# mrsaraei/ViT-2SPN

Measured on NVIDIA B200. Metric: dual-view SSP pairs/sec, ViT-Tiny b128/GPU, higher is better.
Workload: dtype bf16

## Files before the change

### vit-2spn_b200/csrc/common.cuh

```cuda
#pragma once
#include <cuda_bf16.h>
#include <cuda_fp16.h>
#include <cuda_runtime.h>
#include <stdint.h>
#include <string.h>

#include <utility>

#include "../../include/vit2spn.h"

namespace v2s {

typedef __nv_bfloat16 bf16;
typedef __half f16;
constexpr int AT_F32 = 0, AT_BF16 = 1, AT_F16 = 2;

constexpr int D = V2S_HIDDEN;
constexpr int NT = V2S_TOKENS;
constexpr int NP = V2S_PATCHES;
constexpr int NH = V2S_HEADS;
constexpr int DH = V2S_HEAD_DIM;
constexpr int DF = V2S_MLP;
constexpr int NL = V2S_LAYERS;
constexpr int KPE = V2S_PATCH_K;
// ... 64 lines not shown
      v2s::set_error("%s failed: %s (%s:%d)", #expr, cudaGetErrorString(_e), __FILE__, __LINE__); \
      return 1;                                                                               \
    }                                                                                         \
  } while (0)

#define V2S_LAUNCH_CHECK()                                                                    \
  do {                                                                                        \
    ++v2s::g_launch_count;                                                                    \
    cudaError_t _e = cudaGetLastError();                                                      \
    if (_e != cudaSuccess) {                                                                  \
      v2s::set_error("kernel launch failed: %s (%s:%d)", cudaGetErrorString(_e), __FILE__, __LINE__); \
      return 1;                                                                               \
    }                                                                                         \
  } while (0)

#define V2S_TRY(expr)             \
  do {                            \
    int _r = (expr);              \
    if (_r != 0) return _r;       \
  } while (0)

template <typename... KArgs, typename... Args>
inline cudaError_t launch_pdl(void (*kernel)(KArgs...), dim3 grid, dim3 block, size_t smem, cudaStream_t stream,
                              Args&&... args) {
  cudaLaunchConfig_t cfg;
  memset(&cfg, 0, sizeof(cfg));
  cfg.gridDim = grid; cfg.blockDim = block; cfg.dynamicSmemBytes = smem; cfg.stream = stream;
  cudaLaunchAttribute attr[1];
  attr[0].id = cudaLaunchAttributeProgrammaticStreamSerialization;
  attr[0].val.programmaticStreamSerializationAllowed = 1;
  cfg.attrs = attr; cfg.numAttrs = 1;
  return cudaLaunchKernelEx(&cfg, kernel, std::forward<Args>(args)...);
}

template <typename T> __device__ __forceinline__ float to_f(T v);
template <> __device__ __forceinline__ float to_f<float>(float v) { return v; }
template <> __device__ __forceinline__ float to_f<bf16>(bf16 v) { return __bfloat162float(v); }
template <> __device__ __forceinline__ float to_f<f16>(f16 v) { return __half2float(v); }
template <typename T> __device__ __forceinline__ T from_f(float v);
template <> __device__ __forceinline__ float from_f<float>(float v) { return v; }
template <> __device__ __forceinline__ bf16 from_f<bf16>(float v) { return __float2bfloat16_rn(v); }
template <> __device__ __forceinline__ f16 from_f<f16>(float v) { return __float2half_rn(v); }

__device__ __forceinline__ float warp_sum(float v) {
#pragma unroll
  for (int o = 16; o > 0; o >>= 1) v += __shfl_xor_sync(0xffffffffu, v, o);
  return v;
}
__device__ __forceinline__ float warp_max(float v) {
#pragma unroll
  for (int o = 16; o > 0; o >>= 1) v = fmaxf(v, __shfl_xor_sync(0xffffffffu, v, o));
  return v;
}

__device__ __forceinline__ float gelu_f(float x) { return 0.5f * x * (1.0f + erff(x * 0.70710678118654752f)); }
__device__ __forceinline__ float gelu_grad_f(float x) {
  const float cdf = 0.5f * (1.0f + erff(x * 0.70710678118654752f));
  const float pdf = 0.39894228040143268f * __expf(-0.5f * x * x);
  return cdf + x * pdf;
}

template <typename T> struct GPtr {
  T* p[MAXG];
};

}
// ... 1 lines not shown
```

### vit-2spn_b200/csrc/mlp_tc.cu

```cuda
#include <string.h>

#include "gemm_tc.cuh"
#include "mlp_tc.cuh"
#include "ptx.cuh"
#include "tc_math.cuh"

namespace v2s {

namespace {

constexpr int BM = 128;
constexpr int CW = 64;
constexpr int NCH = DF / CW;
constexpr int KB1 = D / 64;
constexpr int KBLK = BM * 128;
constexpr int A1_BYTES = KB1 * KBLK;
constexpr int SW = 2 * CW;
constexpr int NSC = DF / SW;
constexpr int W_SLOT = 24576;
constexpr int W_SLOTS = 3;
constexpr int OFF_W = A1_BYTES;
constexpr int N_EB = 6;
constexpr int OFF_EB = OFF_W + W_SLOTS * W_SLOT;
constexpr int OFF_BAR = OFF_EB + N_EB * KBLK;
constexpr int SMEM_BYTES = OFF_BAR + 1024 + 1024;
constexpr int TM_ACC2 = 128;
constexpr int N_THREADS = 768;
constexpr int GELU_THREADS = 512;
constexpr int DRAIN_THREADS = 128;
constexpr int XCH = D / 32;
static_assert(SMEM_BYTES <= 232448, "shared-memory budget");
static_assert(OFF_W % 1024 == 0 && OFF_EB % 1024 == 0 && W_SLOT % 1024 == 0, "swizzled tiles need 1024-byte alignment");
static_assert(NCH % 2 == 0, "per-buffer phase bookkeeping assumes an even number of chunks per tile");

struct alignas(64) MlpParams {
  CUtensorMap tmA[MAXG], tmB1[MAXG], tmB2[MAXG];
  CUtensorMap tmH[MAXG];
  CUtensorMap tmU[MAXG];
  CUtensorMap tmRes[MAXG];
  CUtensorMap tmOut[MAXG];
  CUtensorMap tmXn[MAXG];
  const float* b1[MAXG]; const float* b2[MAXG];
  const float* ln_gamma[MAXG]; const float* ln_beta[MAXG]; float* ln_mean[MAXG]; float* ln_rstd[MAXG];
  int has_h[MAXG], has_u[MAXG], has_ln[MAXG];
  int M, tiles_m, total_tiles, late_wait;
  int* err_flag;
  long long* dbg;
};

template <int MODE, typename LP, bool DBG>
__global__ void __launch_bounds__(N_THREADS, 1) mlp_tc_kernel(const __grid_constant__ MlpParams p) {
  extern __shared__ uint8_t smem_raw[];
  uint8_t* smem = reinterpret_cast<uint8_t*>((reinterpret_cast<uintptr_t>(smem_raw) + 1023) & ~uintptr_t(1023));
  uint64_t* a1_full = reinterpret_cast<uint64_t*>(smem + OFF_BAR);
  uint64_t* a1_empty = a1_full + 1;
  uint64_t* w_full = a1_empty + 1;
  uint64_t* w_empty = w_full + W_SLOTS;
  uint64_t* acc1_full = w_empty + W_SLOTS;
  uint64_t* acc1_empty = acc1_full + 2;
  uint64_t* a2_full = acc1_empty + 2;
  uint64_t* a2_free = a2_full + 2;
  uint64_t* u_full = a2_free + 2;
  uint64_t* u_free = u_full + 2;
  uint64_t* acc2_full = u_free + 2;
  uint64_t* acc2_empty = acc2_full + 2;
  uint64_t* rs_full = acc2_empty + 2;
  uint64_t* dst_full = rs_full + 2;
  uint64_t* dbuf_free = dst_full + 2;
  uint32_t* tmem_ptr = reinterpret_cast<uint32_t*>(dbuf_free + 2);

  const int warp = __shfl_sync(0xffffffffu, threadIdx.x >> 5, 0), lane = threadIdx.x & 31;

  if (warp == 0 && lane == 0) {
    for (int g = 0; g * p.tiles_m < p.total_tiles; ++g) {
      ptx::prefetch_tmap(&p.tmA[g]); ptx::prefetch_tmap(&p.tmB1[g]); ptx::prefetch_tmap(&p.tmB2[g]);
    }
  }
  if (warp == 1 && lane == 0) {
    ptx::mbar_init(a1_full, 1); ptx::mbar_init(a1_empty, 1);
    for (int s = 0; s < W_SLOTS; ++s) { ptx::mbar_init(&w_full[s], 1); ptx::mbar_init(&w_empty[s], 1); }
    for (int s = 0; s < 2; ++s) {
      ptx::mbar_init(&acc1_full[s], 1); ptx::mbar_init(&acc1_empty[s], 16);
      ptx::mbar_init(&a2_full[s], GELU_THREADS); ptx::mbar_init(&a2_free[s], 2);
      ptx::mbar_init(&u_full[s], MODE == MLP_FWD ? GELU_THREADS : 1);
      ptx::mbar_init(&u_free[s], MODE == MLP_FWD ? 1 : GELU_THREADS);
      ptx::mbar_init(&acc2_full[s], 1); ptx::mbar_init(&acc2_empty[s], 4);
      ptx::mbar_init(&rs_full[s], 1); ptx::mbar_init(&dst_full[s], DRAIN_THREADS); ptx::mbar_init(&dbuf_free[s], 1);
    }
    ptx::fence_barrier_init();
  }
  if (warp == 2) {
    ptx::tmem_alloc(tmem_ptr, 512);
    ptx::tmem_relinquish();
  }
  ptx::tc_fence_before();
  __syncthreads();
  ptx::tc_fence_after();
  const uint32_t tmem_base = __shfl_sync(0xffffffffu, *tmem_ptr, 0);
  if (!p.late_wait) {
    ptx::pdl_wait();
    ptx::pdl_launch_dependents();
  }

  const int n_my = ((int)blockIdx.x < p.total_tiles) ? (p.total_tiles - 1 - (int)blockIdx.x) / (int)gridDim.x + 1 : 0;
  auto tile_at = [&](int i, int& g, int& mt) {
    const int t = blockIdx.x + i * gridDim.x;
    g = t / p.tiles_m;
    mt = t - g * p.tiles_m;
  };
  uint8_t* const eb = smem + OFF_EB;
  long long tk[8] = {0, 0, 0, 0, 0, 0, 0, 0};
  const long long t_begin = DBG ? clock64() : 0;
#define V2S_WAIT(slot, bar, par, code)                                   \
  do {                                                                  \
    const long long _t0 = DBG ? clock64() : 0;                          \
    ptx::mbar_wait(bar, par, p.err_flag, code);                         \
    if (DBG) tk[slot] += clock64() - _t0;                               \
  } while (0)

  if (warp == 0) {
    int ws = 0; uint32_t wph = 0;
    auto advance = [&]() { if (++ws == W_SLOTS) { ws = 0; wph ^= 1; } };
    auto load_b1 = [&](int g, int k) {
#pragma unroll 1
      for (int kb = 0; kb < KB1; ++kb) {
        ptx::mbar_wait(&w_empty[ws], wph ^ 1, p.err_flag, 41);
        if (ptx::elect_one()) {
          uint8_t* slot = smem + OFF_W + ws * W_SLOT;
          ptx::mbar_arrive_expect_tx(&w_full[ws], SW * 128);
          if (MODE == MLP_FWD) {
            ptx::tma_load_2d(slot, &p.tmB1[g], &w_full[ws], kb * 64, k * SW);
          } else {
            ptx::tma_load_2d(slot, &p.tmB1[g], &w_full[ws], k * SW, kb * 64);
            ptx::tma_load_2d(slot + 8192, &p.tmB1[g], &w_full[ws], k * SW + 64, kb * 64);
          }
        }
        __syncwarp();
        advance();
      }
    };
    auto load_b2 = [&](int g, int j) {
      ptx::mbar_wait(&w_empty[ws], wph ^ 1, p.err_flag, 42);
      if (ptx::elect_one()) {
        uint8_t* slot = smem + OFF_W + ws * W_SLOT;
        ptx::mbar_arrive_expect_tx(&w_full[ws], W_SLOT);
        if (MODE == MLP_FWD) {
          ptx::tma_load_2d(slot, &p.tmB2[g], &w_full[ws], j * CW, 0);
        } else {
          ptx::tma_load_2d(slot, &p.tmB2[g], &w_full[ws], 0, j * CW);
          ptx::tma_load_2d(slot + 8192, &p.tmB2[g], &w_full[ws], 64, j * CW);
          ptx::tma_load_2d(slot + 16384, &p.tmB2[g], &w_full[ws], 128, j * CW);
        }
      }
      __syncwarp();
      advance();
    };
    auto load_a1 = [&](int i) {
      int g, mt;
      tile_at(i, g, mt);
      ptx::mbar_wait(a1_empty, (i & 1) ^ 1, p.err_flag, 43);
      if (ptx::elect_one()) {
        ptx::mbar_arrive_expect_tx(a1_full, A1_BYTES);
#pragma unroll
        for (int kb = 0; kb < KB1; ++kb) ptx::tma_load_2d(smem + kb * KBLK, &p.tmA[g], a1_full, kb * 64, mt * BM);
      }
      __syncwarp();
    };
    const int n_sc = n_my * NSC;
    auto grp = [&](int K) { int g, mt; tile_at(K / NSC, g, mt); return g; };
    if (n_sc > 0) { load_a1(0); load_b1(grp(0), 0); }
#pragma unroll 1
    for (int K = 0; K < n_sc; ++K) {
      if (K >= 1) load_b2(grp(K - 1), 2 * ((K - 1) % NSC) + 1);
      if (K + 1 < n_sc) {
        if ((K + 1) % NSC == 0) load_a1((K + 1) / NSC);
        load_b1(grp(K + 1), (K + 1) % NSC);
      }
      load_b2(grp(K), 2 * (K % NSC));
    }
    if (n_sc > 0) load_b2(grp(n_sc - 1), 2 * ((n_sc - 1) % NSC) + 1);
  } else if (warp == 1) {
    constexpr uint32_t b_mn = (MODE == MLP_BWD) ? 1u : 0u;
    const uint32_t idesc2 = make_idesc_lp(LP::kIdescFmt, BM, D, 0, b_mn);
    const uint32_t sbase = ptx::smem_u32(smem);
    const uint32_t b_lbo = b_mn ? 8192u : 16u, b_step = b_mn ? (2048u >> 4) : (32u >> 4);
    int ws = 0; uint32_t wph = 0;
    auto advance = [&]() { if (++ws == W_SLOTS) { ws = 0; wph ^= 1; } };
    const uint32_t idesc1 = make_idesc_lp(LP::kIdescFmt, BM, SW, 0, b_mn);
    auto stage1 = [&](int K) {
      const int i = K / NSC, k = K - i * NSC;
      V2S_WAIT(0, acc1_empty, (K & 1) ^ 1, 44);
      if (k == 0) V2S_WAIT(1, a1_full, i & 1, 45);
#pragma unroll 1
      for (int kb = 0; kb < KB1; ++kb) {
        V2S_WAIT(2, &w_full[ws], wph, 46);
        ptx::tc_fence_after();
        const uint32_t a_lo = ptx::desc_lo(sbase + kb * KBLK, 16);
        const uint32_t b_lo = ptx::desc_lo(sbase + OFF_W + ws * W_SLOT, b_lbo);
        if (ptx::elect_one()) {
#pragma unroll
          for (int kk = 0; kk < 4; ++kk)
            ptx::umma_bf16_lohi(tmem_base, a_lo + kk * 2, b_lo + kk * b_step, ptx::DESC_HI_SW128_SBO1024, idesc1,
                                (kb > 0 || kk > 0) ? 1u : 0u);
          ptx::umma_commit(&w_empty[ws]);
          if (kb == KB1 - 1) {
            ptx::umma_commit(acc1_full);
            if (k == NSC - 1) ptx::umma_commit(a1_empty);
          }
        }
        __syncwarp();
        advance();
      }
    };
    auto stage2 = [&](int c) {
      const int i = c / NCH, j = c - i * NCH;
      const int s = i & 1, b = c & 1;
      if (j == 0) V2S_WAIT(3, &acc2_empty[s], ((i >> 1) & 1) ^ 1, 47);
      V2S_WAIT(4, &a2_full[b], (c >> 1) & 1, 48);
      V2S_WAIT(5, &w_full[ws], wph, 49);
      ptx::tc_fence_after();
      const uint32_t d_tmem = tmem_base + TM_ACC2 + s * D;
      const uint32_t a_lo = ptx::desc_lo(sbase + OFF_EB + b * KBLK, 16);
      const uint32_t b_lo = ptx::desc_lo(sbase + OFF_W + ws * W_SLOT, b_lbo);
      if (ptx::elect_one()) {
#pragma unroll
        for (int kk = 0; kk < 4; ++kk)
          ptx::umma_bf16_lohi(d_tmem, a_lo + kk * 2, b_lo + kk * b_step, ptx::DESC_HI_SW128_SBO1024, idesc2,
                              (j > 0 || kk > 0) ? 1u : 0u);
        ptx::umma_commit(&w_empty[ws]);
        ptx::umma_commit(&a2_free[b]);
        if (j == NCH - 1) ptx::umma_commit(&acc2_full[s]);
      }
      __syncwarp();
      advance();
    };
    const int n_sc = n_my * NSC;
    if (n_sc > 0) stage1(0);
#pragma unroll 1
    for (int K = 0; K < n_sc; ++K) {
      if (K >= 1) stage2(2 * K - 1);
      if (K + 1 < n_sc) stage1(K + 1);
      stage2(2 * K);
    }
    if (n_sc > 0) stage2(2 * n_sc - 1);
    if (DBG && blockIdx.x == 0 && lane == 0) {
      for (int k = 0; k < 6; ++k) p.dbg[k] = tk[k];
      p.dbg[6] = clock64() - t_begin; p.dbg[7] = n_my;
    }
  } else if (warp == 2) {
    int c = 0, nut = 0;
    const int n_chunks = n_my * NCH;
    auto load_u = [&](int cc) {
      const int ti = cc / NCH, jj = cc - ti * NCH;
      int g2, mt2;
      tile_at(ti, g2, mt2);
      ptx::mbar_arrive_expect_tx(&u_full[cc & 1], KBLK);
      ptx::tma_load_2d(eb + (2 + (cc & 1)) * KBLK, &p.tmU[g2], &u_full[cc & 1], jj * CW, mt2 * BM);
    };
    if (MODE == MLP_BWD && lane == 0) {
      if (n_chunks > 0) load_u(0);
      if (n_chunks > 1) load_u(1);
    }
    __syncwarp();
    for (int i = 0; i < n_my; ++i) {
      int g, mt;
      tile_at(i, g, mt);
      const int m0 = mt * BM;
      const bool has_h = p.has_h[g] != 0, has_u = MODE == MLP_FWD && p.has_u[g] != 0;
      const bool stores = has_h || has_u;
#pragma unroll 1
      for (int j = 0; j < NCH; ++j, ++c) {
        const int b = c & 1;
        if (MODE == MLP_BWD && c + 2 < n_chunks) {
          ptx::mbar_wait(&u_free[b], (c >> 1) & 1, p.err_flag, 53);
          if (lane == 0) load_u(c + 2);
          __syncwarp();
        }
        ptx::mbar_wait(&a2_full[b], (c >> 1) & 1, p.err_flag, 54);
        if (has_u) ptx::mbar_wait(&u_full[b], (nut * (NCH / 2) + (j >> 1)) & 1, p.err_flag, 55);
        if (lane == 0) {
          if (stores) {
            if (has_h) ptx::tma_store_2d(&p.tmH[g], eb + b * KBLK, j * CW, m0);
            if (has_u) ptx::tma_store_2d(&p.tmU[g], eb + (2 + b) * KBLK, j * CW, m0);
            ptx::tma_commit_group();
            if (j > 0) {
              ptx::tma_wait_group_read<1>();
              ptx::mbar_arrive(&a2_free[b ^ 1]);
              if (has_u) ptx::mbar_arrive(&u_free[b ^ 1]);
            }
            if (j == NCH - 1) {
              ptx::tma_wait_group_read<0>();
              ptx::mbar_arrive(&a2_free[b]);
              if (has_u) ptx::mbar_arrive(&u_free[b]);
            }
          } else {
            ptx::mbar_arrive(&a2_free[b]);
          }
        }
        __syncwarp();
      }
      if (has_u) ++nut;
    }
    if (lane == 0) ptx::tma_wait_group<0>();
    __syncwarp();
  } else if (warp == 3) {
    int use0 = 0, use1 = 0;
    auto load_res = [&](int ti, int k) {
      int g2, mt2;
      tile_at(ti, g2, mt2);
      ptx::mbar_arrive_expect_tx(&rs_full[k & 1], KBLK);
      ptx::tma_load_2d(eb + (4 + (k & 1)) * KBLK, &p.tmRes[g2], &rs_full[k & 1], k * 32, mt2 * BM);
    };
    if (MODE == MLP_FWD && n_my > 0 && lane == 0) { load_res(0, 0); load_res(0, 1); }
    __syncwarp();
    for (int i = 0; i < n_my; ++i) {
      int g, mt;
      tile_at(i, g, mt);
      const int m0 = mt * BM;
      const int n_out = MODE == MLP_FWD ? XCH : 0;
      const int n_lp = MODE == MLP_FWD ? (p.has_ln[g] != 0 ? 3 : 0) : 3;
      const int n_all = n_out + n_lp;
#pragma unroll 1
      for (int k = 0; k < n_all; ++k) {
        const int t = k - n_out;
        const int b = (k < n_out ? k : t) & 1;
        ptx::mbar_wait(&dst_full[b], (b ? use1 : use0) & 1, p.err_flag, 57);
        if (lane == 0) {
          if (k < n_out) ptx::tma_store_2d(&p.tmOut[g], eb + (4 + b) * KBLK, k * 32, m0);
          else ptx::tma_store_2d(MODE == MLP_FWD ? &p.tmXn[g] : &p.tmOut[g], eb + (4 + b) * KBLK, t * 64, m0);
          ptx::tma_commit_group();
          ptx::tma_wait_group_read<0>();
          ptx::mbar_arrive(&dbuf_free[b]);
          if (MODE == MLP_FWD) {
            if (k + 2 < n_out) load_res(i, k + 2);
            else if (i + 1 < n_my) {
              const bool last_use = n_lp == 0 ? true : (b == 0 ? t == 2 : t == 1);
              if (last_use) load_res(i + 1, b);
            }
          }
        }
        __syncwarp();
        use0 += b ^ 1; use1 += b;
      }
    }
    if (lane == 0) ptx::tma_wait_group<0>();
    __syncwarp();
  } else if (warp >= 4 && warp < 20) {
    const int q = warp & 3;
    const int cq = (warp - 4) >> 2;
    const int row = q * 32 + lane;
    const int rx = row & 7;
    const uint32_t tl = tmem_base + ((uint32_t)(q * 32) << 16);
    const uint32_t eb_row = ptx::smem_u32(eb) + row * 128;
    const uint32_t pc0 = ((2 * cq) ^ rx) << 4, pc1 = ((2 * cq + 1) ^ rx) << 4;
    int c = 0, nut = 0;
    uint32_t rr[32];
    for (int i = 0; i < n_my; ++i) {
      int g, mt;
      tile_at(i, g, mt);
      const bool has_u = MODE == MLP_FWD && p.has_u[g] != 0;
#pragma unroll 1
      for (int j = 0; j < NCH; ++j, ++c) {
        const int b = c & 1;
        uint4 ux0, ux1;
        if (MODE == MLP_BWD) {
          V2S_WAIT(0, &u_full[b], (c >> 1) & 1, 61);
          ux0 = ptx::lds128(eb_row + (2 + b) * KBLK + pc0);
          ux1 = ptx::lds128(eb_row + (2 + b) * KBLK + pc1);
          __threadfence_block();
          ptx::mbar_arrive(&u_free[b]);
        }
        if (b == 0) {
          V2S_WAIT(1, acc1_full, (c >> 1) & 1, 50);
          ptx::tc_fence_after();
          ptx::tmem_ld_32x16(tl + cq * 16, rr);
          ptx::tmem_ld_32x16(tl + CW + cq * 16, rr + 16);
          ptx::tmem_ld_wait();
          ptx::tc_fence_before();
          if (lane == 0) ptx::mbar_arrive(acc1_empty);
        }
        uint32_t r[16];
#pragma unroll
        for (int e = 0; e < 16; ++e) r[e] = b ? rr[16 + e] : rr[e];
        uint32_t o[8], pu[8];
        if (MODE == MLP_FWD) {
          const float4* b4 = reinterpret_cast<const float4*>(p.b1[g] + j * CW + cq * 16);
          float v[16];
#pragma unroll
          for (int t = 0; t < 4; ++t) {
            const float4 bb = __ldg(b4 + t);
            v[4 * t] = __uint_as_float(r[4 * t]) + bb.x; v[4 * t + 1] = __uint_as_float(r[4 * t + 1]) + bb.y;
            v[4 * t + 2] = __uint_as_float(r[4 * t + 2]) + bb.z; v[4 * t + 3] = __uint_as_float(r[4 * t + 3]) + bb.w;
          }
          if (has_u) {
#pragma unroll
            for (int k = 0; k < 8; ++k) pu[k] = LP::pack(v[2 * k], v[2 * k + 1]);
          }
#pragma unroll
          for (int k = 0; k < 8; ++k) o[k] = LP::pack(gelu_fast(v[2 * k]), gelu_fast(v[2 * k + 1]));
        } else {
          const uint32_t w[8] = {ux0.x, ux0.y, ux0.z, ux0.w, ux1.x, ux1.y, ux1.z, ux1.w};
#pragma unroll
          for (int e = 0; e < 8; ++e)
            o[e] = LP::pack(__uint_as_float(r[2 * e]) * gelu_grad_fast(LP::lo(w[e])),
                            __uint_as_float(r[2 * e + 1]) * gelu_grad_fast(LP::hi(w[e])));
        }
        V2S_WAIT(2, &a2_free[b], ((c >> 1) & 1) ^ 1, 51);
        ptx::sts128(eb_row + b * KBLK + pc0, o[0], o[1], o[2], o[3]);
        ptx::sts128(eb_row + b * KBLK + pc1, o[4], o[5], o[6], o[7]);
        if (has_u) {
          V2S_WAIT(3, &u_free[b], ((nut * (NCH / 2) + (j >> 1)) & 1) ^ 1, 62);
          ptx::sts128(eb_row + (2 + b) * KBLK + pc0, pu[0], pu[1], pu[2], pu[3]);
          ptx::sts128(eb_row + (2 + b) * KBLK + pc1, pu[4], pu[5], pu[6], pu[7]);
          ptx::fence_proxy_async();
          ptx::mbar_arrive(&a2_full[b]);
          ptx::mbar_arrive(&u_full[b]);
        } else {
          ptx::fence_proxy_async();
          ptx::mbar_arrive(&a2_full[b]);
        }
      }
      if (has_u) ++nut;
    }
    if (DBG && blockIdx.x == 0 && threadIdx.x == 128) {
      for (int k = 0; k < 4; ++k) p.dbg[8 + k] = tk[k];
      p.dbg[12] = clock64() - t_begin;
    }
  } else if (warp >= 20 && warp < 24) {
    const int q = warp & 3;
    const int row = q * 32 + lane;
    const int rx = row & 7;
    const uint32_t tl = tmem_base + ((uint32_t)(q * 32) << 16) + TM_ACC2;
    const uint32_t eb_row = ptx::smem_u32(eb) + 4 * KBLK + row * 128;
    int use0 = 0, use1 = 0, nres0 = 0, nres1 = 0;
    for (int i = 0; i < n_my; ++i) {
      int g, mt;
      tile_at(i, g, mt);
      const int s = i & 1;
      const int64_t grow = (int64_t)mt * BM + row;
      const uint32_t ta = tl + s * D;
      V2S_WAIT(4, &acc2_full[s], (i >> 1) & 1, 52);
      const long long t_d0 = DBG ? clock64() : 0;
      ptx::tc_fence_after();
      if (MODE == MLP_FWD) {
        const bool has_ln = p.has_ln[g] != 0;
        float s1 = 0.f, s2 = 0.f;
#pragma unroll 1
        for (int k = 0; k < XCH; ++k) {
          const int b = k & 1;
          uint32_t r[32];
          ptx::tmem_ld_32x32(ta + k * 32, r);
          const float4* b4 = reinterpret_cast<const float4*>(p.b2[g] + k * 32);
          V2S_WAIT(5, &rs_full[b], (b ? nres1 : nres0) & 1, 63);
// ... 49 lines not shown
              }
            }
            ptx::fence_proxy_async();
            ptx::mbar_arrive(&dst_full[b]);
            use0 += b ^ 1; use1 += b;
          }
        }
      } else {
#pragma unroll 1
        for (int t = 0; t < 3; ++t) {
          const int b = t & 1;
          const uint32_t sb = eb_row + b * KBLK;
#pragma unroll 1
          for (int hf = 0; hf < 2; ++hf) {
            uint32_t r[32];
            ptx::tmem_ld_32x32(ta + t * 64 + hf * 32, r);
            if (hf == 0) V2S_WAIT(6, &dbuf_free[b], ((b ? use1 : use0) & 1) ^ 1, 65);
            ptx::tmem_ld_wait();
#pragma unroll
            for (int e = 0; e < 4; ++e) {
              const uint32_t* x = r + 8 * e;
              ptx::sts128(sb + (((hf * 4 + e) ^ rx) << 4), LP::pack(__uint_as_float(x[0]), __uint_as_float(x[1])),
                          LP::pack(__uint_as_float(x[2]), __uint_as_float(x[3])), LP::pack(__uint_as_float(x[4]), __uint_as_float(x[5])),
                          LP::pack(__uint_as_float(x[6]), __uint_as_float(x[7])));
            }
          }
          ptx::fence_proxy_async();
          ptx::mbar_arrive(&dst_full[b]);
          use0 += b ^ 1; use1 += b;
        }
      }
      ptx::tc_fence_before();
      __syncwarp();
      if (lane == 0) ptx::mbar_arrive(&acc2_empty[s]);
      if (DBG) tk[7] += clock64() - t_d0;
    }
    if (DBG && blockIdx.x == 0 && threadIdx.x == 640) {
      p.dbg[13] = tk[4]; p.dbg[14] = tk[5]; p.dbg[15] = tk[6]; p.dbg[16] = tk[7];
      p.dbg[17] = clock64() - t_begin;
    }
  }
#undef V2S_WAIT

  if (p.late_wait) { ptx::pdl_wait(); ptx::pdl_launch_dependents(); }
  ptx::tc_fence_before();
  __syncthreads();
  if (warp == 2) {
    ptx::tc_fence_after();
    ptx::tmem_dealloc(tmem_base, 512);
  }
}

template <int MODE, typename LP>
int launch_impl(const MlpParams& p, int grid, cudaStream_t stream) {
  static bool attr_set[MAX_DEVICES] = {false};
  if (!attr_set[cur_device()]) {
    V2S_CUDA_OK(cudaFuncSetAttribute(mlp_tc_kernel<MODE, LP, false>, cudaFuncAttributeMaxDynamicSharedMemorySize, SMEM_BYTES));
    V2S_CUDA_OK(cudaFuncSetAttribute(mlp_tc_kernel<MODE, LP, true>, cudaFuncAttributeMaxDynamicSharedMemorySize, SMEM_BYTES));
    attr_set[cur_device()] = true;
  }
  if (p.dbg) V2S_CUDA_OK(launch_pdl(mlp_tc_kernel<MODE, LP, true>, dim3(grid), dim3(N_THREADS), (size_t)SMEM_BYTES, stream, p));
  else V2S_CUDA_OK(launch_pdl(mlp_tc_kernel<MODE, LP, false>, dim3(grid), dim3(N_THREADS), (size_t)SMEM_BYTES, stream, p));
  V2S_LAUNCH_CHECK();
  return 0;
}

}

int launch_mlp_tc(const MlpDesc& d, cudaStream_t stream) {
  if (d.groups < 1 || d.groups > MAXG || d.M < 1) { set_error("mlp_tc: bad shape"); return 1; }
  MlpParams p;
  memset(&p, 0, sizeof(p));
  p.M = d.M;
  p.tiles_m = (d.M + BM - 1) / BM;
  p.total_tiles = p.tiles_m * d.groups;
  p.late_wait = d.late_wait ? 1 : 0;
  p.err_flag = tc_err_flag();
  p.dbg = tc_dbg_counters();
  for (int g = 0; g < d.groups; ++g) {
    if (!d.a[g] || !d.w1[g] || !d.w2[g] || !d.out[g]) { set_error("mlp_tc: null operand (group %d)", g); return 1; }
    V2S_TRY(tmap_get_2d(&p.tmA[g], d.a[g], D, d.M, D, 64, BM, true, 128));
    if (d.mode == MLP_FWD) {
      if (!d.b1[g] || !d.b2[g] || !d.resid[g]) { set_error("mlp_tc: forward needs biases and the residual"); return 1; }
      V2S_TRY(tmap_get_2d(&p.tmB1[g], d.w1[g], D, DF, D, 64, SW, true, 128));
      V2S_TRY(tmap_get_2d(&p.tmB2[g], d.w2[g], DF, D, DF, 64, D, true, 128));
      V2S_TRY(tmap_get_2d(&p.tmRes[g], d.resid[g], D, d.M, D, 32, BM, false, 128));
      V2S_TRY(tmap_get_2d(&p.tmOut[g], d.out[g], D, d.M, D, 32, BM, false, 128));
      if (d.h[g]) { V2S_TRY(tmap_get_2d(&p.tmH[g], d.h[g], DF, d.M, DF, 64, BM, true, 128)); p.has_h[g] = 1; }
      if (d.u[g]) { V2S_TRY(tmap_get_2d(&p.tmU[g], d.u[g], DF, d.M, DF, 64, BM, true, 128)); p.has_u[g] = 1; }
      if (d.ln_out[g]) {
        if (!d.ln_gamma[g] || !d.ln_beta[g]) { set_error("mlp_tc: fused LayerNorm needs gamma and beta"); return 1; }
        V2S_TRY(tmap_get_2d(&p.tmXn[g], d.ln_out[g], D, d.M, D, 64, BM, true, 128));
        p.has_ln[g] = 1;
      }
    } else {
      if (!d.u[g] || !d.h[g]) { set_error("mlp_tc: backward needs u and the du buffer"); return 1; }
      V2S_TRY(tmap_get_2d(&p.tmB1[g], d.w2[g], DF, D, DF, 64, 64, true, 128));
      V2S_TRY(tmap_get_2d(&p.tmB2[g], d.w1[g], D, DF, D, 64, 64, true, 128));
      V2S_TRY(tmap_get_2d(&p.tmH[g], d.h[g], DF, d.M, DF, 64, BM, true, 128));
      V2S_TRY(tmap_get_2d(&p.tmU[g], d.u[g], DF, d.M, DF, 64, BM, true, 128));
      V2S_TRY(tmap_get_2d(&p.tmOut[g], d.out[g], D, d.M, D, 64, BM, true, 128));
      p.has_h[g] = 1; p.has_u[g] = 1;
    }
    p.b1[g] = d.b1[g]; p.b2[g] = d.b2[g];
    p.ln_gamma[g] = d.ln_gamma[g]; p.ln_beta[g] = d.ln_beta[g]; p.ln_mean[g] = d.ln_mean[g]; p.ln_rstd[g] = d.ln_rstd[g];
  }
  const int sms = tc_num_sms();
  const int grid = p.total_tiles < sms ? p.total_tiles : sms;
  if (d.mode == MLP_FWD)
    return d.lp_f16 ? launch_impl<MLP_FWD, LpF16>(p, grid, stream) : launch_impl<MLP_FWD, LpBf16>(p, grid, stream);
  return d.lp_f16 ? launch_impl<MLP_BWD, LpF16>(p, grid, stream) : launch_impl<MLP_BWD, LpBf16>(p, grid, stream);
}

}
```

### vit-2spn_b200/csrc/ptx.cuh

```cuda
#pragma once
#include <cuda.h>
#include <cuda_runtime.h>
#include <stdint.h>

namespace v2s {
namespace ptx {

__device__ __forceinline__ uint32_t smem_u32(const void* p) {
  return static_cast<uint32_t>(__cvta_generic_to_shared(p));
}

__device__ __forceinline__ bool elect_one() {
  uint32_t pred = 0;
  asm volatile(
      "{\n\t.reg .pred P;\n\t.reg .b32 R;\n\t"
      "elect.sync R|P, 0xffffffff;\n\t"
      "selp.u32 %0, 1, 0, P;\n\t}\n"
      : "=r"(pred));
  return pred != 0;
}

__device__ __forceinline__ void mbar_init(uint64_t* bar, uint32_t count) {
  asm volatile("mbarrier.init.shared::cta.b64 [%0], %1;" ::"r"(smem_u32(bar)), "r"(count) : "memory");
}
// ... 120 lines not shown
                                          uint32_t accumulate) {
  asm volatile(
      "{\n\t.reg .pred p;\n\t"
      "setp.ne.b32 p, %4, 0;\n\t"
      "tcgen05.mma.cta_group::1.kind::f16 [%0], %1, %2, %3, p;\n\t}\n"
      ::"r"(tmem_d), "l"(desc_a), "l"(desc_b), "r"(idesc), "r"(accumulate)
      : "memory");
}
__device__ __forceinline__ void umma_bf16_lohi(uint32_t tmem_d, uint32_t a_lo, uint32_t b_lo, uint32_t desc_hi,
                                               uint32_t idesc, uint32_t accumulate) {
  asm volatile(
      "{\n\t.reg .pred p;\n\t.reg .b64 da, db;\n\t"
      "setp.ne.b32 p, %5, 0;\n\t"
      "mov.b64 da, {%1, %3};\n\t"
      "mov.b64 db, {%2, %3};\n\t"
      "tcgen05.mma.cta_group::1.kind::f16 [%0], da, db, %4, p;\n\t}\n"
      ::"r"(tmem_d), "r"(a_lo), "r"(b_lo), "r"(desc_hi), "r"(idesc), "r"(accumulate)
      : "memory");
}
__device__ __forceinline__ void umma_bf16_ts(uint32_t tmem_d, uint32_t tmem_a, uint32_t b_lo, uint32_t desc_hi,
                                             uint32_t idesc, uint32_t accumulate) {
  asm volatile(
      "{\n\t.reg .pred p;\n\t.reg .b64 db;\n\t"
      "setp.ne.b32 p, %5, 0;\n\t"
      "mov.b64 db, {%2, %3};\n\t"
      "tcgen05.mma.cta_group::1.kind::f16 [%0], [%1], db, %4, p;\n\t}\n"
      ::"r"(tmem_d), "r"(tmem_a), "r"(b_lo), "r"(desc_hi), "r"(idesc), "r"(accumulate)
      : "memory");
}
__device__ __forceinline__ uint32_t desc_lo(uint32_t smem_addr, uint32_t lbo_bytes) {
  return ((smem_addr & 0x3FFFF) >> 4) | ((lbo_bytes >> 4) << 16);
}
constexpr uint32_t DESC_HI_SW128_SBO1024 = (1024u >> 4) | (1u << 14) | (2u << 29);

__device__ __forceinline__ void umma_commit(uint64_t* bar) {
  asm volatile("tcgen05.commit.cta_group::1.mbarrier::arrive::one.shared::cluster.b64 [%0];" ::"r"(smem_u32(bar))
               : "memory");
}

__device__ __forceinline__ void tmem_ld_32x32(uint32_t taddr, uint32_t* r) {
  asm volatile(
      "tcgen05.ld.sync.aligned.32x32b.x32.b32 "
      "{%0, %1, %2, %3, %4, %5, %6, %7, %8, %9, %10, %11, %12, %13, %14, %15, "
      "%16, %17, %18, %19, %20, %21, %22, %23, %24, %25, %26, %27, %28, %29, %30, %31}, [%32];"
      : "=r"(r[0]), "=r"(r[1]), "=r"(r[2]), "=r"(r[3]), "=r"(r[4]), "=r"(r[5]), "=r"(r[6]), "=r"(r[7]), "=r"(r[8]),
        "=r"(r[9]), "=r"(r[10]), "=r"(r[11]), "=r"(r[12]), "=r"(r[13]), "=r"(r[14]), "=r"(r[15]), "=r"(r[16]),
        "=r"(r[17]), "=r"(r[18]), "=r"(r[19]), "=r"(r[20]), "=r"(r[21]), "=r"(r[22]), "=r"(r[23]), "=r"(r[24]),
        "=r"(r[25]), "=r"(r[26]), "=r"(r[27]), "=r"(r[28]), "=r"(r[29]), "=r"(r[30]), "=r"(r[31])
      : "r"(taddr)
      : "memory");
}
__device__ __forceinline__ void tmem_ld_32x16(uint32_t taddr, uint32_t* r) {
  asm volatile(
      "tcgen05.ld.sync.aligned.32x32b.x16.b32 "
      "{%0, %1, %2, %3, %4, %5, %6, %7, %8, %9, %10, %11, %12, %13, %14, %15}, [%16];"
      : "=r"(r[0]), "=r"(r[1]), "=r"(r[2]), "=r"(r[3]), "=r"(r[4]), "=r"(r[5]), "=r"(r[6]), "=r"(r[7]), "=r"(r[8]),
        "=r"(r[9]), "=r"(r[10]), "=r"(r[11]), "=r"(r[12]), "=r"(r[13]), "=r"(r[14]), "=r"(r[15])
      : "r"(taddr)
      : "memory");
}
__device__ __forceinline__ void tmem_ld_32x8(uint32_t taddr, uint32_t* r) {
  asm volatile(
      "tcgen05.ld.sync.aligned.32x32b.x8.b32 {%0, %1, %2, %3, %4, %5, %6, %7}, [%8];"
      : "=r"(r[0]), "=r"(r[1]), "=r"(r[2]), "=r"(r[3]), "=r"(r[4]), "=r"(r[5]), "=r"(r[6]), "=r"(r[7])
      : "r"(taddr)
      : "memory");
}
__device__ __forceinline__ void tmem_st_32x32(uint32_t taddr, const uint32_t* r) {
  asm volatile(
// ... 65 lines not shown
```

Measured before the change: 18620.

## Convert fused MLP kernel to 2-CTA cluster tcgen05 MMA with split weight loads

Switches the fused MLP tensor-core kernel to CTA pairs: each cluster of two CTAs issues cta_group::2 UMMAs with M=256, and each CTA loads half of every weight tile through pair TMA, halving per-CTA weight smem traffic. Barriers are re-plumbed to arrive on the leader CTA, and weight slots are resized to twice as many half-size slots. It also adds TMA L2 prefetches for the next A tile, upcoming U chunks and the residual. The change brings cluster scheduling constraints, extra cross-CTA synchronisation, and a pair-level job split that can leave one CTA idle when the tile count is odd.

```diff
diff --git a/vit-2spn_b200/csrc/common.cuh b/vit-2spn_b200/csrc/common.cuh
--- a/vit-2spn_b200/csrc/common.cuh
+++ b/vit-2spn_b200/csrc/common.cuh
@@ -120,6 +120,20 @@
   cfg.attrs = attr; cfg.numAttrs = 1;
   return cudaLaunchKernelEx(&cfg, kernel, std::forward<Args>(args)...);
 }
+template <typename... KArgs, typename... Args>
+inline cudaError_t launch_pdl_cluster(void (*kernel)(KArgs...), int cluster_x, dim3 grid, dim3 block, size_t smem,
+                                      cudaStream_t stream, Args&&... args) {
+  cudaLaunchConfig_t cfg;
+  memset(&cfg, 0, sizeof(cfg));
+  cfg.gridDim = grid; cfg.blockDim = block; cfg.dynamicSmemBytes = smem; cfg.stream = stream;
+  cudaLaunchAttribute attr[2];
+  attr[0].id = cudaLaunchAttributeProgrammaticStreamSerialization;
+  attr[0].val.programmaticStreamSerializationAllowed = 1;
+  attr[1].id = cudaLaunchAttributeClusterDimension;
+  attr[1].val.clusterDim.x = cluster_x; attr[1].val.clusterDim.y = 1; attr[1].val.clusterDim.z = 1;
+  cfg.attrs = attr; cfg.numAttrs = 2;
+  return cudaLaunchKernelEx(&cfg, kernel, std::forward<Args>(args)...);
+}
 
 template <typename T> __device__ __forceinline__ float to_f(T v);
 template <> __device__ __forceinline__ float to_f<float>(float v) { return v; }
diff --git a/vit-2spn_b200/csrc/mlp_tc.cu b/vit-2spn_b200/csrc/mlp_tc.cu
--- a/vit-2spn_b200/csrc/mlp_tc.cu
+++ b/vit-2spn_b200/csrc/mlp_tc.cu
@@ -17,8 +17,10 @@
 constexpr int A1_BYTES = KB1 * KBLK;
 constexpr int SW = 2 * CW;
 constexpr int NSC = DF / SW;
-constexpr int W_SLOT = 24576;
-constexpr int W_SLOTS = 3;
+constexpr int W_SLOT = 12288;
+constexpr int W_SLOTS = 6;
+constexpr int W1_HALF = SW / 2 * 128;
+constexpr int W2_HALF = D / 2 * 128;
 constexpr int OFF_W = A1_BYTES;
 constexpr int N_EB = 6;
 constexpr int OFF_EB = OFF_W + W_SLOTS * W_SLOT;
@@ -43,7 +45,7 @@
   const float* b1[MAXG]; const float* b2[MAXG];
   const float* ln_gamma[MAXG]; const float* ln_beta[MAXG]; float* ln_mean[MAXG]; float* ln_rstd[MAXG];
   int has_h[MAXG], has_u[MAXG], has_ln[MAXG];
-  int M, tiles_m, total_tiles, late_wait;
+  int M, tiles_m, pairs_m, total_jobs, late_wait;
   int* err_flag;
   long long* dbg;
 };
@@ -67,12 +69,15 @@
   uint64_t* rs_full = acc2_empty + 2;
   uint64_t* dst_full = rs_full + 2;
   uint64_t* dbuf_free = dst_full + 2;
-  uint32_t* tmem_ptr = reinterpret_cast<uint32_t*>(dbuf_free + 2);
+  uint64_t* a2_pair = dbuf_free + 2;
+  uint32_t* tmem_ptr = reinterpret_cast<uint32_t*>(a2_pair + 2);
+  const uint32_t rank = ptx::cluster_ctarank();
+  constexpr uint16_t PAIR_MASK = 0x3;
 
   const int warp = __shfl_sync(0xffffffffu, threadIdx.x >> 5, 0), lane = threadIdx.x & 31;
 
   if (warp == 0 && lane == 0) {
-    for (int g = 0; g * p.tiles_m < p.total_tiles; ++g) {
+    for (int g = 0; g * p.pairs_m < p.total_jobs; ++g) {
       ptx::prefetch_tmap(&p.tmA[g]); ptx::prefetch_tmap(&p.tmB1[g]); ptx::prefetch_tmap(&p.tmB2[g]);
     }
   }
@@ -80,21 +85,22 @@
     ptx::mbar_init(a1_full, 1); ptx::mbar_init(a1_empty, 1);
     for (int s = 0; s < W_SLOTS; ++s) { ptx::mbar_init(&w_full[s], 1); ptx::mbar_init(&w_empty[s], 1); }
     for (int s = 0; s < 2; ++s) {
-      ptx::mbar_init(&acc1_full[s], 1); ptx::mbar_init(&acc1_empty[s], 16);
+      ptx::mbar_init(&acc1_full[s], 1); ptx::mbar_init(&acc1_empty[s], 2 * 16);
       ptx::mbar_init(&a2_full[s], GELU_THREADS); ptx::mbar_init(&a2_free[s], 2);
       ptx::mbar_init(&u_full[s], MODE == MLP_FWD ? GELU_THREADS : 1);
       ptx::mbar_init(&u_free[s], MODE == MLP_FWD ? 1 : GELU_THREADS);
-      ptx::mbar_init(&acc2_full[s], 1); ptx::mbar_init(&acc2_empty[s], 4);
+      ptx::mbar_init(&acc2_full[s], 1); ptx::mbar_init(&acc2_empty[s], 2 * 4);
       ptx::mbar_init(&rs_full[s], 1); ptx::mbar_init(&dst_full[s], DRAIN_THREADS); ptx::mbar_init(&dbuf_free[s], 1);
+      ptx::mbar_init(&a2_pair[s], 2 * 16);
     }
     ptx::fence_barrier_init();
   }
   if (warp == 2) {
-    ptx::tmem_alloc(tmem_ptr, 512);
-    ptx::tmem_relinquish();
+    ptx::tmem_alloc_pair(tmem_ptr, 512);
+    ptx::tmem_relinquish_pair();
   }
   ptx::tc_fence_before();
-  __syncthreads();
+  ptx::cluster_sync();
   ptx::tc_fence_after();
   const uint32_t tmem_base = __shfl_sync(0xffffffffu, *tmem_ptr, 0);
   if (!p.late_wait) {
@@ -102,11 +108,12 @@
     ptx::pdl_launch_dependents();
   }
 
-  const int n_my = ((int)blockIdx.x < p.total_tiles) ? (p.total_tiles - 1 - (int)blockIdx.x) / (int)gridDim.x + 1 : 0;
+  const int pair = blockIdx.x >> 1, n_pairs = gridDim.x >> 1;
+  const int n_my = (pair < p.total_jobs) ? (p.total_jobs - 1 - pair) / n_pairs + 1 : 0;
   auto tile_at = [&](int i, int& g, int& mt) {
-    const int t = blockIdx.x + i * gridDim.x;
-    g = t / p.tiles_m;
-    mt = t - g * p.tiles_m;
+    const int t = pair + i * n_pairs;
+    g = t / p.pairs_m;
+    mt = 2 * (t - g * p.pairs_m) + (int)rank;
   };
   uint8_t* const eb = smem + OFF_EB;
   long long tk[8] = {0, 0, 0, 0, 0, 0, 0, 0};
@@ -121,18 +128,19 @@
   if (warp == 0) {
     int ws = 0; uint32_t wph = 0;
     auto advance = [&]() { if (++ws == W_SLOTS) { ws = 0; wph ^= 1; } };
+    auto w_full_l = [&](int s) { return ptx::mapa_shared(&w_full[s], 0); };
     auto load_b1 = [&](int g, int k) {
 #pragma unroll 1
       for (int kb = 0; kb < KB1; ++kb) {
         ptx::mbar_wait(&w_empty[ws], wph ^ 1, p.err_flag, 41);
         if (ptx::elect_one()) {
           uint8_t* slot = smem + OFF_W + ws * W_SLOT;
-          ptx::mbar_arrive_expect_tx(&w_full[ws], SW * 128);
+          if (rank == 0) ptx::mbar_arrive_expect_tx(&w_full[ws], 2 * W1_HALF);
+          const int n0 = k * SW + (int)rank * (SW / 2);
           if (MODE == MLP_FWD) {
-            ptx::tma_load_2d(slot, &p.tmB1[g], &w_full[ws], kb * 64, k * SW);
+            ptx::tma_load_2d_pair(slot, &p.tmB1[g], w_full_l(ws), kb * 64, n0);
           } else {
-            ptx::tma_load_2d(slot, &p.tmB1[g], &w_full[ws], k * SW, kb * 64);
-            ptx::tma_load_2d(slot + 8192, &p.tmB1[g], &w_full[ws], k * SW + 64, kb * 64);
+            ptx::tma_load_2d_pair(slot, &p.tmB1[g], w_full_l(ws), n0, kb * 64);
           }
         }
         __syncwarp();
@@ -143,13 +151,14 @@
       ptx::mbar_wait(&w_empty[ws], wph ^ 1, p.err_flag, 42);
       if (ptx::elect_one()) {
         uint8_t* slot = smem + OFF_W + ws * W_SLOT;
-        ptx::mbar_arrive_expect_tx(&w_full[ws], W_SLOT);
+        if (rank == 0) ptx::mbar_arrive_expect_tx(&w_full[ws], 2 * W2_HALF);
+        const int n0 = (int)rank * (D / 2);
         if (MODE == MLP_FWD) {
-          ptx::tma_load_2d(slot, &p.tmB2[g], &w_full[ws], j * CW, 0);
+          ptx::tma_load_2d_pair(slot, &p.tmB2[g], w_full_l(ws), j * CW, n0);
         } else {
-          ptx::tma_load_2d(slot, &p.tmB2[g], &w_full[ws], 0, j * CW);
-          ptx::tma_load_2d(slot + 8192, &p.tmB2[g], &w_full[ws], 64, j * CW);
-          ptx::tma_load_2d(slot + 16384, &p.tmB2[g], &w_full[ws], 128, j * CW);
+          ptx::tma_load_2d_pair(slot, &p.tmB2[g], w_full_l(ws), n0, j * CW);
+          ptx::tma_load_2d_pair(slot + 4096, &p.tmB2[g], w_full_l(ws), n0 + 32, j * CW);
+          ptx::tma_load_2d_pair(slot + 8192, &p.tmB2[g], w_full_l(ws), n0 + 64, j * CW);
         }
       }
       __syncwarp();
@@ -160,9 +169,10 @@
       tile_at(i, g, mt);
       ptx::mbar_wait(a1_empty, (i & 1) ^ 1, p.err_flag, 43);
       if (ptx::elect_one()) {
-        ptx::mbar_arrive_expect_tx(a1_full, A1_BYTES);
-#pragma unroll
-        for (int kb = 0; kb < KB1; ++kb) ptx::tma_load_2d(smem + kb * KBLK, &p.tmA[g], a1_full, kb * 64, mt * BM);
+        if (rank == 0) ptx::mbar_arrive_expect_tx(a1_full, 2 * A1_BYTES);
+        const uint32_t bar = ptx::mapa_shared(a1_full, 0);
+#pragma unroll
+        for (int kb = 0; kb < KB1; ++kb) ptx::tma_load_2d_pair(smem + kb * KBLK, &p.tmA[g], bar, kb * 64, mt * BM);
       }
       __syncwarp();
     };
@@ -171,6 +181,13 @@
     if (n_sc > 0) { load_a1(0); load_b1(grp(0), 0); }
 #pragma unroll 1
     for (int K = 0; K < n_sc; ++K) {
+      if (K % NSC == 0 && K / NSC + 1 < n_my && lane == 0) {
+        int g, mt;
+        tile_at(K / NSC + 1, g, mt);
+#pragma unroll
+        for (int kb = 0; kb < KB1; ++kb) ptx::tma_prefetch_2d(&p.tmA[g], kb * 64, mt * BM);
+      }
+      __syncwarp();
       if (K >= 1) load_b2(grp(K - 1), 2 * ((K - 1) % NSC) + 1);
       if (K + 1 < n_sc) {
         if ((K + 1) % NSC == 0) load_a1((K + 1) / NSC);
@@ -179,14 +196,22 @@
       load_b2(grp(K), 2 * (K % NSC));
     }
     if (n_sc > 0) load_b2(grp(n_sc - 1), 2 * ((n_sc - 1) % NSC) + 1);
-  } else if (warp == 1) {
+#pragma unroll 1
+    for (int s = 0; s < W_SLOTS; ++s) {
+      ptx::mbar_wait(&w_empty[ws], wph ^ 1, p.err_flag, 40);
+      advance();
+    }
+    ptx::mbar_wait(a1_empty, (n_my & 1) ^ 1, p.err_flag, 40);
+  } else if (warp == 1 && rank == 0) {
     constexpr uint32_t b_mn = (MODE == MLP_BWD) ? 1u : 0u;
-    const uint32_t idesc2 = make_idesc_lp(LP::kIdescFmt, BM, D, 0, b_mn);
     const uint32_t sbase = ptx::smem_u32(smem);
-    const uint32_t b_lbo = b_mn ? 8192u : 16u, b_step = b_mn ? (2048u >> 4) : (32u >> 4);
+    const uint32_t b1_lbo = b_mn ? 8192u : 16u, b1_step = b_mn ? (2048u >> 4) : (32u >> 4);
+    const uint32_t b2_lbo = b_mn ? 4096u : 16u, b2_step = b_mn ? (1024u >> 4) : (32u >> 4);
+    const uint32_t b2_hi = b_mn ? ptx::DESC_HI_SW64_SBO512 : ptx::DESC_HI_SW128_SBO1024;
     int ws = 0; uint32_t wph = 0;
     auto advance = [&]() { if (++ws == W_SLOTS) { ws = 0; wph ^= 1; } };
-    const uint32_t idesc1 = make_idesc_lp(LP::kIdescFmt, BM, SW, 0, b_mn);
+    const uint32_t idesc1 = make_idesc_lp(LP::kIdescFmt, 2 * BM, SW, 0, b_mn);
+    const uint32_t idesc2 = make_idesc_lp(LP::kIdescFmt, 2 * BM, D, 0, b_mn);
     auto stage1 = [&](int K) {
       const int i = K / NSC, k = K - i * NSC;
       V2S_WAIT(0, acc1_empty, (K & 1) ^ 1, 44);
@@ -196,16 +221,16 @@
         V2S_WAIT(2, &w_full[ws], wph, 46);
         ptx::tc_fence_after();
         const uint32_t a_lo = ptx::desc_lo(sbase + kb * KBLK, 16);
-        const uint32_t b_lo = ptx::desc_lo(sbase + OFF_W + ws * W_SLOT, b_lbo);
+        const uint32_t b_lo = ptx::desc_lo(sbase + OFF_W + ws * W_SLOT, b1_lbo);
         if (ptx::elect_one()) {
 #pragma unroll
           for (int kk = 0; kk < 4; ++kk)
-            ptx::umma_bf16_lohi(tmem_base, a_lo + kk * 2, b_lo + kk * b_step, ptx::DESC_HI_SW128_SBO1024, idesc1,
-                                (kb > 0 || kk > 0) ? 1u : 0u);
-          ptx::umma_commit(&w_empty[ws]);
+            ptx::umma_pair_lohi(tmem_base, a_lo + kk * 2, ptx::DESC_HI_SW128_SBO1024, b_lo + kk * b1_step,
+                                ptx::DESC_HI_SW128_SBO1024, idesc1, (kb > 0 || kk > 0) ? 1u : 0u);
+          ptx::umma_commit_pair(&w_empty[ws], PAIR_MASK);
           if (kb == KB1 - 1) {
-            ptx::umma_commit(acc1_full);
-            if (k == NSC - 1) ptx::umma_commit(a1_empty);
+            ptx::umma_commit_pair(acc1_full, PAIR_MASK);
+            if (k == NSC - 1) ptx::umma_commit_pair(a1_empty, PAIR_MASK);
           }
         }
         __syncwarp();
@@ -216,20 +241,20 @@
       const int i = c / NCH, j = c - i * NCH;
       const int s = i & 1, b = c & 1;
       if (j == 0) V2S_WAIT(3, &acc2_empty[s], ((i >> 1) & 1) ^ 1, 47);
-      V2S_WAIT(4, &a2_full[b], (c >> 1) & 1, 48);
+      V2S_WAIT(4, &a2_pair[b], (c >> 1) & 1, 48);
       V2S_WAIT(5, &w_full[ws], wph, 49);
       ptx::tc_fence_after();
       const uint32_t d_tmem = tmem_base + TM_ACC2 + s * D;
       const uint32_t a_lo = ptx::desc_lo(sbase + OFF_EB + b * KBLK, 16);
-      const uint32_t b_lo = ptx::desc_lo(sbase + OFF_W + ws * W_SLOT, b_lbo);
+      const uint32_t b_lo = ptx::desc_lo(sbase + OFF_W + ws * W_SLOT, b2_lbo);
       if (ptx::elect_one()) {
 #pragma unroll
         for (int kk = 0; kk < 4; ++kk)
-          ptx::umma_bf16_lohi(d_tmem, a_lo + kk * 2, b_lo + kk * b_step, ptx::DESC_HI_SW128_SBO1024, idesc2,
+          ptx::umma_pair_lohi(d_tmem, a_lo + kk * 2, ptx::DESC_HI_SW128_SBO1024, b_lo + kk * b2_step, b2_hi, idesc2,
                               (j > 0 || kk > 0) ? 1u : 0u);
-        ptx::umma_commit(&w_empty[ws]);
-        ptx::umma_commit(&a2_free[b]);
-        if (j == NCH - 1) ptx::umma_commit(&acc2_full[s]);
+        ptx::umma_commit_pair(&w_empty[ws], PAIR_MASK);
+        ptx::umma_commit_pair(&a2_free[b], PAIR_MASK);
+        if (j == NCH - 1) ptx::umma_commit_pair(&acc2_full[s], PAIR_MASK);
       }
       __syncwarp();
       advance();
@@ -273,7 +298,15 @@
         const int b = c & 1;
         if (MODE == MLP_BWD && c + 2 < n_chunks) {
           ptx::mbar_wait(&u_free[b], (c >> 1) & 1, p.err_flag, 53);
-          if (lane == 0) load_u(c + 2);
+          if (lane == 0) {
+            load_u(c + 2);
+            if (c + 6 < n_chunks) {
+              const int ti = (c + 6) / NCH;
+              int g2, mt2;
+              tile_at(ti, g2, mt2);
+              ptx::tma_prefetch_2d(&p.tmU[g2], (c + 6 - ti * NCH) * CW, mt2 * BM);
+            }
+          }
           __syncwarp();
         }
         ptx::mbar_wait(&a2_full[b], (c >> 1) & 1, p.err_flag, 54);
@@ -301,6 +334,7 @@
       }
       if (has_u) ++nut;
     }
+    for (int cc = n_chunks; cc < n_chunks + 2; ++cc) ptx::mbar_wait(&a2_free[cc & 1], ((cc >> 1) & 1) ^ 1, p.err_flag, 56);
     if (lane == 0) ptx::tma_wait_group<0>();
     __syncwarp();
   } else if (warp == 3) {
@@ -317,6 +351,12 @@
       int g, mt;
       tile_at(i, g, mt);
       const int m0 = mt * BM;
+      if (MODE == MLP_FWD && i + 1 < n_my && lane == 0) {
+        int g2, mt2;
+        tile_at(i + 1, g2, mt2);
+        for (int k = 0; k < XCH; ++k) ptx::tma_prefetch_2d(&p.tmRes[g2], k * 32, mt2 * BM);
+      }
+      __syncwarp();
       const int n_out = MODE == MLP_FWD ? XCH : 0;
       const int n_lp = MODE == MLP_FWD ? (p.has_ln[g] != 0 ? 3 : 0) : 3;
       const int n_all = n_out + n_lp;
@@ -377,7 +417,7 @@
           ptx::tmem_ld_32x16(tl + CW + cq * 16, rr + 16);
           ptx::tmem_ld_wait();
           ptx::tc_fence_before();
-          if (lane == 0) ptx::mbar_arrive(acc1_empty);
+          if (lane == 0) ptx::mbar_arrive_cluster(ptx::mapa_shared(acc1_empty, 0));
         }
         uint32_t r[16];
 #pragma unroll
@@ -419,6 +459,8 @@
           ptx::fence_proxy_async();
           ptx::mbar_arrive(&a2_full[b]);
         }
+        __syncwarp();
+        if (lane == 0) ptx::mbar_arrive_cluster(ptx::mapa_shared(&a2_pair[b], 0));
       }
       if (has_u) ++nut;
     }
@@ -534,7 +576,7 @@
       }
       ptx::tc_fence_before();
       __syncwarp();
-      if (lane == 0) ptx::mbar_arrive(&acc2_empty[s]);
+      if (lane == 0) ptx::mbar_arrive_cluster(ptx::mapa_shared(&acc2_empty[s], 0));
       if (DBG) tk[7] += clock64() - t_d0;
     }
     if (DBG && blockIdx.x == 0 && threadIdx.x == 640) {
@@ -546,23 +588,39 @@
 
   if (p.late_wait) { ptx::pdl_wait(); ptx::pdl_launch_dependents(); }
   ptx::tc_fence_before();
-  __syncthreads();
+  ptx::cluster_sync();
   if (warp == 2) {
     ptx::tc_fence_after();
-    ptx::tmem_dealloc(tmem_base, 512);
+    ptx::tmem_dealloc_pair(tmem_base, 512);
   }
 }
 
 template <int MODE, typename LP>
-int launch_impl(const MlpParams& p, int grid, cudaStream_t stream) {
-  static bool attr_set[MAX_DEVICES] = {false};
-  if (!attr_set[cur_device()]) {
+int launch_impl(const MlpParams& p, cudaStream_t stream) {
+  static int max_pairs[MAX_DEVICES] = {0};
+  const int dev = cur_device();
+  if (max_pairs[dev] == 0) {
     V2S_CUDA_OK(cudaFuncSetAttribute(mlp_tc_kernel<MODE, LP, false>, cudaFuncAttributeMaxDynamicSharedMemorySize, SMEM_BYTES));
     V2S_CUDA_OK(cudaFuncSetAttribute(mlp_tc_kernel<MODE, LP, true>, cudaFuncAttributeMaxDynamicSharedMemorySize, SMEM_BYTES));
-    attr_set[cur_device()] = true;
-  }
-  if (p.dbg) V2S_CUDA_OK(launch_pdl(mlp_tc_kernel<MODE, LP, true>, dim3(grid), dim3(N_THREADS), (size_t)SMEM_BYTES, stream, p));
-  else V2S_CUDA_OK(launch_pdl(mlp_tc_kernel<MODE, LP, false>, dim3(grid), dim3(N_THREADS), (size_t)SMEM_BYTES, stream, p));
+    cudaLaunchConfig_t cfg;
+    memset(&cfg, 0, sizeof(cfg));
+    cfg.gridDim = dim3(2); cfg.blockDim = dim3(N_THREADS); cfg.dynamicSmemBytes = SMEM_BYTES;
+    cudaLaunchAttribute attr[1];
+    attr[0].id = cudaLaunchAttributeClusterDimension;
+    attr[0].val.clusterDim.x = 2; attr[0].val.clusterDim.y = 1; attr[0].val.clusterDim.z = 1;
+    cfg.attrs = attr; cfg.numAttrs = 1;
+    int n = 0;
+    V2S_CUDA_OK(cudaOccupancyMaxActiveClusters(&n, mlp_tc_kernel<MODE, LP, false>, &cfg));
+    if (n < 1) { set_error("mlp_tc: no CTA pair fits on this device"); return 1; }
+    max_pairs[dev] = n;
+  }
+  int pairs = tc_num_sms() / 2;
+  if (pairs > max_pairs[dev]) pairs = max_pairs[dev];
+  if (pairs > p.total_jobs) pairs = p.total_jobs;
+  if (pairs < 1) pairs = 1;
+  const dim3 grid(2 * pairs);
+  if (p.dbg) V2S_CUDA_OK(launch_pdl_cluster(mlp_tc_kernel<MODE, LP, true>, 2, grid, dim3(N_THREADS), (size_t)SMEM_BYTES, stream, p));
+  else V2S_CUDA_OK(launch_pdl_cluster(mlp_tc_kernel<MODE, LP, false>, 2, grid, dim3(N_THREADS), (size_t)SMEM_BYTES, stream, p));
   V2S_LAUNCH_CHECK();
   return 0;
 }
@@ -575,7 +633,8 @@
   memset(&p, 0, sizeof(p));
   p.M = d.M;
   p.tiles_m = (d.M + BM - 1) / BM;
-  p.total_tiles = p.tiles_m * d.groups;
+  p.pairs_m = (p.tiles_m + 1) / 2;
+  p.total_jobs = p.pairs_m * d.groups;
   p.late_wait = d.late_wait ? 1 : 0;
   p.err_flag = tc_err_flag();
   p.dbg = tc_dbg_counters();
@@ -584,8 +643,8 @@
     V2S_TRY(tmap_get_2d(&p.tmA[g], d.a[g], D, d.M, D, 64, BM, true, 128));
     if (d.mode == MLP_FWD) {
       if (!d.b1[g] || !d.b2[g] || !d.resid[g]) { set_error("mlp_tc: forward needs biases and the residual"); return 1; }
-      V2S_TRY(tmap_get_2d(&p.tmB1[g], d.w1[g], D, DF, D, 64, SW, true, 128));
-      V2S_TRY(tmap_get_2d(&p.tmB2[g], d.w2[g], DF, D, DF, 64, D, true, 128));
+      V2S_TRY(tmap_get_2d(&p.tmB1[g], d.w1[g], D, DF, D, 64, SW / 2, true, 128));
+      V2S_TRY(tmap_get_2d(&p.tmB2[g], d.w2[g], DF, D, DF, 64, D / 2, true, 128));
       V2S_TRY(tmap_get_2d(&p.tmRes[g], d.resid[g], D, d.M, D, 32, BM, false, 128));
       V2S_TRY(tmap_get_2d(&p.tmOut[g], d.out[g], D, d.M, D, 32, BM, false, 128));
       if (d.h[g]) { V2S_TRY(tmap_get_2d(&p.tmH[g], d.h[g], DF, d.M, DF, 64, BM, true, 128)); p.has_h[g] = 1; }
@@ -598,7 +657,7 @@
     } else {
       if (!d.u[g] || !d.h[g]) { set_error("mlp_tc: backward needs u and the du buffer"); return 1; }
       V2S_TRY(tmap_get_2d(&p.tmB1[g], d.w2[g], DF, D, DF, 64, 64, true, 128));
-      V2S_TRY(tmap_get_2d(&p.tmB2[g], d.w1[g], D, DF, D, 64, 64, true, 128));
+      V2S_TRY(tmap_get_2d(&p.tmB2[g], d.w1[g], D, DF, D, 32, 64, true, 64));
       V2S_TRY(tmap_get_2d(&p.tmH[g], d.h[g], DF, d.M, DF, 64, BM, true, 128));
       V2S_TRY(tmap_get_2d(&p.tmU[g], d.u[g], DF, d.M, DF, 64, BM, true, 128));
       V2S_TRY(tmap_get_2d(&p.tmOut[g], d.out[g], D, d.M, D, 64, BM, true, 128));
@@ -607,11 +666,9 @@
     p.b1[g] = d.b1[g]; p.b2[g] = d.b2[g];
     p.ln_gamma[g] = d.ln_gamma[g]; p.ln_beta[g] = d.ln_beta[g]; p.ln_mean[g] = d.ln_mean[g]; p.ln_rstd[g] = d.ln_rstd[g];
   }
-  const int sms = tc_num_sms();
-  const int grid = p.total_tiles < sms ? p.total_tiles : sms;
   if (d.mode == MLP_FWD)
-    return d.lp_f16 ? launch_impl<MLP_FWD, LpF16>(p, grid, stream) : launch_impl<MLP_FWD, LpBf16>(p, grid, stream);
-  return d.lp_f16 ? launch_impl<MLP_BWD, LpF16>(p, grid, stream) : launch_impl<MLP_BWD, LpBf16>(p, grid, stream);
+    return d.lp_f16 ? launch_impl<MLP_FWD, LpF16>(p, stream) : launch_impl<MLP_FWD, LpBf16>(p, stream);
+  return d.lp_f16 ? launch_impl<MLP_BWD, LpF16>(p, stream) : launch_impl<MLP_BWD, LpBf16>(p, stream);
 }
 
 }
diff --git a/vit-2spn_b200/csrc/ptx.cuh b/vit-2spn_b200/csrc/ptx.cuh
--- a/vit-2spn_b200/csrc/ptx.cuh
+++ b/vit-2spn_b200/csrc/ptx.cuh
@@ -176,9 +176,60 @@
   return ((smem_addr & 0x3FFFF) >> 4) | ((lbo_bytes >> 4) << 16);
 }
 constexpr uint32_t DESC_HI_SW128_SBO1024 = (1024u >> 4) | (1u << 14) | (2u << 29);
+constexpr uint32_t DESC_HI_SW64_SBO512 = (512u >> 4) | (1u << 14) | (4u << 29);
 
 __device__ __forceinline__ void umma_commit(uint64_t* bar) {
   asm volatile("tcgen05.commit.cta_group::1.mbarrier::arrive::one.shared::cluster.b64 [%0];" ::"r"(smem_u32(bar))
+               : "memory");
+}
+
+__device__ __forceinline__ uint32_t cluster_ctarank() {
+  uint32_t r;
+  asm volatile("mov.u32 %0, %%cluster_ctarank;" : "=r"(r));
+  return r;
+}
+__device__ __forceinline__ void cluster_sync() {
+  asm volatile("barrier.cluster.arrive.release.aligned;\n\tbarrier.cluster.wait.acquire.aligned;" ::: "memory");
+}
+__device__ __forceinline__ uint32_t mapa_shared(const void* p, uint32_t rank) {
+  uint32_t a;
+  asm volatile("mapa.shared::cluster.u32 %0, %1, %2;" : "=r"(a) : "r"(smem_u32(p)), "r"(rank));
+  return a;
+}
+__device__ __forceinline__ void mbar_arrive_cluster(uint32_t cluster_bar) {
+  asm volatile("mbarrier.arrive.shared::cluster.b64 _, [%0];" ::"r"(cluster_bar) : "memory");
+}
+__device__ __forceinline__ void tma_load_2d_pair(void* smem_dst, const CUtensorMap* m, uint32_t cluster_bar, int c0,
+                                                 int c1) {
+  asm volatile(
+      "cp.async.bulk.tensor.2d.cta_group::2.shared::cluster.global.mbarrier::complete_tx::bytes [%0], [%1, {%3, %4}], [%2];"
+      ::"r"(smem_u32(smem_dst)), "l"(reinterpret_cast<uint64_t>(m)), "r"(cluster_bar), "r"(c0), "r"(c1)
+      : "memory");
+}
+__device__ __forceinline__ void tmem_alloc_pair(uint32_t* smem_dst, uint32_t ncols) {
+  asm volatile("tcgen05.alloc.cta_group::2.sync.aligned.shared::cta.b32 [%0], %1;" ::"r"(smem_u32(smem_dst)), "r"(ncols)
+               : "memory");
+}
+__device__ __forceinline__ void tmem_relinquish_pair() {
+  asm volatile("tcgen05.relinquish_alloc_permit.cta_group::2.sync.aligned;" ::: "memory");
+}
+__device__ __forceinline__ void tmem_dealloc_pair(uint32_t taddr, uint32_t ncols) {
+  asm volatile("tcgen05.dealloc.cta_group::2.sync.aligned.b32 %0, %1;" ::"r"(taddr), "r"(ncols) : "memory");
+}
+__device__ __forceinline__ void umma_pair_lohi(uint32_t tmem_d, uint32_t a_lo, uint32_t a_hi, uint32_t b_lo,
+                                                uint32_t b_hi, uint32_t idesc, uint32_t accumulate) {
+  asm volatile(
+      "{\n\t.reg .pred p;\n\t.reg .b64 da, db;\n\t"
+      "setp.ne.b32 p, %6, 0;\n\t"
+      "mov.b64 da, {%1, %2};\n\t"
+      "mov.b64 db, {%3, %4};\n\t"
+      "tcgen05.mma.cta_group::2.kind::f16 [%0], da, db, %5, p;\n\t}\n"
+      ::"r"(tmem_d), "r"(a_lo), "r"(a_hi), "r"(b_lo), "r"(b_hi), "r"(idesc), "r"(accumulate)
+      : "memory");
+}
+__device__ __forceinline__ void umma_commit_pair(uint64_t* bar, uint16_t cta_mask) {
+  asm volatile("tcgen05.commit.cta_group::2.mbarrier::arrive::one.shared::cluster.multicast::cluster.b64 [%0], %1;"
+               ::"r"(smem_u32(bar)), "h"(cta_mask)
                : "memory");
 }
 
```

Measured after the change: 18870 (median of 6 runs). +1.4%, better.
